# keillernogueira/dynamic-rs-segmentation

Hardware: AMD Instinct MI355X
Metric: training patches/sec dilated_grsl_rate8 64x64x5 (higher is better)
Workload: dtype f32; 1 GPU; dilated_grsl_rate8 (Dilated8Pooling) training step, single_fixed 64x64, 5-band synthetic 2048x2048 tile, global batch 128 (crop+augment+normalise, fwd, loss, bwd, momentum, confusion); global_batch=128, patch=64, bands=5, classes=6, parallelism=dp1, sync_bn=True, rccl_ranks_observed=1

## Files before the change

### dynamic-rs-segmentation_amd/_lib.py

```python
import ctypes as C
import os

_HERE = os.path.dirname(os.path.abspath(__file__))
LIB_PATH = os.path.join(_HERE, "libdrs_hip.so")
DEV_LIB_PATH = os.path.join(_HERE, "libdrs_hip_dev.so")

_p, _i, _f, _d = C.c_void_p, C.c_int, C.c_float, C.c_double
_sz, _u64 = C.c_size_t, C.c_ulonglong

SIGNATURES = {
    "drs_conv_mtile": (_i, [_i]),
    "drs_conv_forward": (_i, [_p, _i, _i, _i, _i, _i, _p, _p, _i, _i, _i, _i, _i, _p, _i, _i, _i, _p, _p]),
    "drs_conv_workspace_floats": (_sz, [_i]),
    "drs_conv_halo_skip": (_i, [_i, _i, _i, _i, _i, _i, _i]),
    "drs_conv_executed_ksteps": (_i, [_i, _i, _i, _i, _i, _i, _i, _p, _p]),
    "drs_conv_forward_ws": (_i, [_p, _i, _i, _i, _i, _i, _p, _p, _i, _i, _i, _i, _i, _p, _i, _i, _i, _p, _p, _sz, _p]),
    "drs_conv_wgrad_splits": (_i, [_i, _i, _i, _i, _i]),
    "drs_conv_wgrad": (_i, [_p, _i, _i, _i, _i, _i, _p, _i, _i, _i, _i, _i, _i, _i, _i, _i, _p, _p, _p]),
    "drs_filter_flip_transpose": (_i, [_p, _p, _i, _i, _i, _p]),
    "drs_filter_pad_cin": (_i, [_p, _p, _i, _i, _i, _i, _p]),
    "drs_split_conv_mtile": (_i, [_i]),
    "drs_split_terms": (_i, [_p, _sz, _i, _p, _p]),
    "drs_filter_split": (_i, [_p, _i, _i, _i, _i, _i, _p, _p, _p]),
    "drs_conv_forward_split": (_i, [_p, _i, _i, _i, _i, _i, _p, _p, _i, _i, _i, _i, _i, _p, _i, _i, _i, _p, _i, _p]),
# ... 91 lines not shown
    "drs_net_se_gate_finish": (_i, [_p, _i, _d, _p]),
    "drs_net_set_two_streams": (_i, [_p, _i]),
    "drs_net_set_class_weights": (_i, [_p, _p, _i]),
    "drs_net_get_class_weights": (_i, [_p, _p, _i, C.POINTER(_i)]),
    "drs_net_set_focal_gamma": (_i, [_p, _f]),
    "drs_net_get_focal_gamma": (_i, [_p, C.POINTER(_f)]),
    "drs_net_timing": (_i, [_p, _i]),
    "drs_net_num_timing_kinds": (_i, []),
    "drs_net_timing_summary": (_i, [_p, _i, C.c_char_p, _i, C.POINTER(_i), C.POINTER(_d), C.POINTER(_d)]),
}
ALLREDUCE_FN = C.CFUNCTYPE(_i, _p, _p, _sz, _i, _i, _p)
WAIT_FN = C.CFUNCTYPE(_i, _p, _i, _p)
WANT_LOGITS, WITH_LABELS, USE_ACC_MASK, USE_LOSS_MASK, NO_UPDATE = 1, 2, 4, 8, 16


DEV_SIGNATURES = {
    "drs_debug_skip_taps": (_i, [_i]), "drs_debug_conv_variant": (_i, [_i]), "drs_debug_conv_wide192": (_i, [_i]),
    "drs_debug_conv_splitk": (_i, [_i]), "drs_debug_conv_hybrid": (_i, [_i]), "drs_debug_conv_sk_order": (_i, [_i]), "drs_debug_conv_prio": (_i, [_i]),
    "drs_debug_conv_sk_geometry": (_i, [_i, _i, _i, _p]), "drs_debug_conv_trace": (_i, [_p]), "drs_debug_conv_lpt": (_i, [_i]), "drs_debug_conv_order": (_i, [_i] * 7 + [_p, _i]),
    "drs_debug_conv_image_tiles": (_i, [_i]), "drs_debug_conv_order_image": (_i, [_i] * 7 + [_p, _i]),
    "drs_debug_wgrad_variant": (_i, [_i]), "drs_debug_wgrad_seg": (_i, [_i]), "drs_debug_wgrad_balance": (_i, [_i]), "drs_debug_wgrad_target": (_i, [_i]),
    "drs_debug_wgrad_target_big": (_i, [_i]), "drs_debug_wgrad_len": (_i, [_i]), "drs_debug_wgrad_minchunks": (_i, [_i]), "drs_debug_wgrad_model": (_i, [_i]), "drs_debug_wgrad_ablate": (_i, [_i]), "drs_debug_wgrad_prio": (_i, [_i]), "drs_debug_cls_variant": (_i, [_i]), "drs_debug_slide_blocks": (_i, [_i]), "drs_debug_slide_minrows": (_i, [_i]), "drs_debug_slide_rowpad": (_i, [_i]), "drs_debug_chain_mode": (_i, [_i]), "drs_debug_jitter": (_i, [C.c_ulonglong]), "drs_debug_wg_stream_prio": (_i, [_i]), "drs_debug_reductions_on_chain": (_i, [_i]), "drs_debug_wgrad_schedule": (_i, [_i, _i, _i]), "drs_debug_variant": (_i, [_i]),
    "drs_debug_wgrad_cut": (_i, [_i] * 7 + [_p, _i, _p, _p]),
}


class DrsError(RuntimeError):
    pass


_lib = None
_dev = None


def _open(path, signatures):
    if not os.path.isfile(path):
        raise DrsError("HIP library not built: %s is missing (run dynamic-rs-segmentation_amd/csrc/build.sh "
                       "or __graft_entry__.build()); there is no CPU fallback" % path)
    import torch
    lib = C.CDLL(path)
    for name, (res, args) in signatures.items():
        fn = getattr(lib, name)
        fn.restype = res
        fn.argtypes = args
    return lib

# ... 49 lines not shown
```

### dynamic-rs-segmentation_amd/csrc/conv_mfma.hip

```cpp
#include "drs_common.hpp"
#include <algorithm>
#include <cstdlib>
#include <map>
#include <mutex>
#include <numeric>
#include <tuple>
#include <vector>

namespace {

constexpr int BK = 32;
constexpr int LDA = BK + 4;

struct ConvArgs {
  const float* in; int S, P, ld_in, coff_in;
  int M;
  const float* w;
  const float* bias;
  float* out; int ld_out, coff_out;
  float* stats;
  int k, rate, pad, Cin, Cout;
  int accumulate;
  int skip_halo;
  float rcpS, rcpSS;
// ... 510 lines not shown
  }
  conv_epilogue<BM, BN, WM, WN>(a, acc, lds, m0, n0);
}

constexpr int WG_MAXT = 64, WG_MAXC = 8;
struct WgradPlan {
  int nclass;
  int n[WG_MAXC];
  int seg_start[WG_MAXC + 1];
  int seg_width[WG_MAXC];
  unsigned char cls[WG_MAXT];
};

struct WgradArgs {
  const float* x; int S, Px, ld_x, coff_x;
  const float* g; int Pg, ld_g, coff_g;
  int M;
  int k, rate, pad, Cin, Cout;
  float* slab;
  int chunks_per_split;
  int ntr, nto;
  int skip_halo;
  int live_cut;
  int prio;
  int ablate;
  float rcpS, rcpSS;
  WgradPlan plan;
#ifdef DRS_DEV
  unsigned long long* trace;
#endif
};

__host__ __device__ __forceinline__ int wave_uniform(int v) {
#if defined(__HIP_DEVICE_COMPILE__)
  return __builtin_amdgcn_readfirstlane(v);
#else
  return v;
#endif
}

__host__ __device__ __forceinline__ void wgrad_assign(const WgradArgs& a, int TR, int id, int& tile, int& split, int& cbeg, int& cend,
                                                      int& live_lo, int& live_hi) {
  const int nchunks_total = (a.M + 31) / 32;
  const int rows_all = a.k * a.k * a.Cin;
  int nr = 0;
  if (a.plan.nclass == 0) {
    const int ntile = a.ntr * a.nto;
    split = id / ntile;
    tile = id % ntile;
  } else {
    int j = 0;
    while (j + 1 < a.plan.nclass && id >= a.plan.seg_start[j + 1]) ++j;
    const int rel = id - a.plan.seg_start[j];
    split = (j ? a.plan.n[j - 1] : 0) + rel / a.plan.seg_width[j];
    const int pos = rel % a.plan.seg_width[j];
    const int want = pos / a.nto;
    int r = 0, seen = 0;
    for (; r < a.ntr; ++r)
      if (a.plan.cls[r] >= j) { if (seen == want) break; ++seen; }
    r = r < a.ntr ? r : a.ntr - 1;
    tile = r * a.nto + pos % a.nto;
    nr = a.plan.n[a.plan.cls[r]];
  }
  tile = wave_uniform(tile);
  split = wave_uniform(split);
  const int R0 = (tile / a.nto) * TR;
  const int rlast = (R0 + TR < rows_all ? R0 + TR : rows_all) - 1;
  int lo, hi;
  live_pixel_range(R0, rlast, a.Cin, a.k, a.rate, a.pad, a.S, a.live_cut, lo, hi);
  if (a.plan.nclass == 0) {
    cbeg = split * a.chunks_per_split;
    cend = cbeg + a.chunks_per_split;
    cend = cend < nchunks_total ? cend : nchunks_total;
  } else {
    const int S2 = a.S * a.S, lp = hi - lo;
    const int live_total = (a.M / S2) * lp;
    const int q = (live_total + nr - 1) / nr;
    auto bound = [&](int s) -> int {
      if (s <= 0) return 0;
      const long long jp = (long long)s * q;
      if (s >= nr || jp >= live_total) return nchunks_total;
      const int img = (int)jp / lp, rem = (int)jp - img * lp;
      return (img * S2 + lo + rem) >> 5;
    };
    cbeg = bound(split);
    cend = bound(split + 1);
  }
  cbeg = wave_uniform(cbeg);
  cend = wave_uniform(cend);
  if (!a.skip_halo) { lo = 0; hi = a.S * a.S; }
  live_lo = lo; live_hi = hi;
}

struct ChunkWalk {
  int c, b, r, y, x0;
  int S, S2, lo, hi, ylo;
  __device__ __forceinline__ void init(int cfirst, int S_, float rcpS, float rcpSS, int lo_, int hi_) {
    S = S_; S2 = S_ * S_; lo = lo_; hi = hi_;
    int q;
    divmod24(lo, S, rcpS, ylo, q);
    c = next_live_chunk(cfirst - 1, S2, rcpSS, lo, hi);
    divmod24(c * 32, S2, rcpSS, b, r);
    divmod24(r, S, rcpS, y, x0);
    c = __builtin_amdgcn_readfirstlane(c); b = __builtin_amdgcn_readfirstlane(b); r = __builtin_amdgcn_readfirstlane(r);
    y = __builtin_amdgcn_readfirstlane(y); x0 = __builtin_amdgcn_readfirstlane(x0); ylo = __builtin_amdgcn_readfirstlane(ylo);
  }
  __device__ __forceinline__ int advance() {
    int r1 = r + 32, b1 = b;
    if (r1 >= S2) { r1 -= S2; ++b1; }
    if ((r1 + 31 >= lo && r1 < hi) || r1 + 31 >= S2 + lo) {
      ++c; r = r1; b = b1;
      x0 += 32;
      if (x0 >= S) { x0 -= S; ++y; }
      if (y >= S) y = 0;
// ... 213 lines not shown
#ifdef DRS_DEV
  if (a.trace && t == 0) a.trace[2 * blockIdx.x + 1] = __builtin_amdgcn_s_memrealtime();
#endif
}

template <int TR, int TO, int MODE>
__global__ __launch_bounds__(64 * (TR >= 64 ? 2 : 1) * (TO >= 64 ? 2 : 1), 3) void wgrad_dma_kernel(const WgradArgs a) {
#if defined(__HIP_DEVICE_COMPILE__)
  constexpr int WR = TR >= 64 ? 2 : 1, WC = TO >= 64 ? 2 : 1;
  constexpr int NW = WR * WC, NT = 64 * NW;
  constexpr int WTR = TR / WR, WTO = TO / WC;
  constexpr int TMr = WTR / 32, TNo = WTO / 32;
  constexpr int BP = 32, HP = 16;
  constexpr int XQ = TR / 4, GQ = TO / 4;
  constexpr int IX = HP * XQ / 64 / NW, IG = HP * GQ / 64 / NW;
  static_assert(IX >= 1 && IG >= 1 && IX * NW * 64 == HP * XQ && IG * NW * 64 == HP * GQ, "tile / wave layout");
  constexpr int XSTAGE = HP * TR, STAGE = HP * (TR + TO);

  __shared__ __attribute__((aligned(1024))) float lds[2 * STAGE];
  __shared__ uint32_t tabx[2][BP], tabg[2][BP];

  constexpr bool AFF = MODE == 1;
  constexpr bool SEG = MODE == 2;
  const int t = threadIdx.x;
  const int lane = t & 63, wave = (AFF || SEG) ? __builtin_amdgcn_readfirstlane(t >> 6) : t >> 6;
  const int li = lane & 31, h = lane >> 5;
  const int wr = wave / WC, wc = wave % WC;

  int tile, split, cbeg, cend, live_lo, live_hi;
#ifdef DRS_DEV
  if (a.trace && t == 0) {
    a.trace[2 * blockIdx.x] = __builtin_amdgcn_s_memrealtime();
    a.trace[32768 + blockIdx.x] = (unsigned long long)__builtin_amdgcn_s_getreg(63492) | ((unsigned long long)__builtin_amdgcn_s_getreg(63508) << 32);
  }
#endif
  wgrad_assign(a, TR, xcd_remap(blockIdx.x, gridDim.x), tile, split, cbeg, cend, live_lo, live_hi);
  const int R0 = (tile / a.nto) * TR;
  const int o0 = (tile % a.nto) * TO;
  const int rows_all = a.k * a.k * a.Cin;
  const int Sxp = a.S + 2 * a.Px, Sgp = a.S + 2 * a.Pg;
  constexpr bool affine = AFF || SEG;
  const int xq = lane % XQ;
  const int myR = R0 + xq * 4;
  const int myRc = myR < rows_all ? myR : 0;
  const int tap = myRc / a.Cin, c0 = myRc % a.Cin;
  const int u = tap / a.k, v = tap % a.k;
  const uint32_t biasx = SEG ? (uint32_t)(32 * a.ld_x) * 4u : 0u, biasg = SEG ? (uint32_t)(32 * a.ld_g) * 4u : 0u;
  const uint32_t xconst = (uint32_t)((a.ablate == 1 ? 0 : (u * a.rate * Sxp + v * a.rate)) * a.ld_x + a.coff_x + c0) * 4u + biasx;
  uint32_t xoff[IX], goff[IG];
  int xpix[IX], gpix[IG];
#pragma unroll
  for (int i = 0; i < IX; ++i) {
    xpix[i] = (64 * (wave + NW * i) + lane) / XQ;
    xoff[i] = xconst + (affine ? (uint32_t)(xpix[i] * a.ld_x) * 4u : 0u);
  }
#pragma unroll
  for (int i = 0; i < IG; ++i) {
    const int f = 64 * (wave + NW * i) + lane;
    gpix[i] = f / GQ;
    goff[i] = (uint32_t)(a.coff_g + o0 + (f % GQ) * 4) * 4u + (affine ? (uint32_t)(gpix[i] * a.ld_g) * 4u : 0u) + biasg;
  }

  f32x16 acc[TMr][TNo];
#pragma unroll
  for (int mi = 0; mi < TMr; ++mi)
#pragma unroll
    for (int ni = 0; ni < TNo; ++ni)
#pragma unroll
      for (int r = 0; r < 16; ++r) acc[mi][ni][r] = 0.f;

  const int nchunks_total = (a.M + BP - 1) / BP;
  const int clast = (a.M & 31) ? nchunks_total - 1 : -1;
  ChunkWalk w;
  w.init(cbeg, a.S, a.rcpS, a.rcpSS, live_lo, live_hi);

  int py = 0, px = 0;
  uint32_t ox = 0, og = 0;
  const uint32_t stepx = (uint32_t)(32 * a.ld_x) * 4u, stepg = (uint32_t)(32 * a.ld_g) * 4u;
  const uint32_t rowjx = (uint32_t)((Sxp - a.S) * a.ld_x) * 4u, rowjg = (uint32_t)((Sgp - a.S) * a.ld_g) * 4u;
  const uint32_t imgjx = (uint32_t)(Sxp * (Sxp - a.S) * a.ld_x) * 4u, imgjg = (uint32_t)(Sgp * (Sgp - a.S) * a.ld_g) * 4u;
  auto pixel_from_index = [&](int p) {
    int pb, rem;
    divmod24(p < a.M ? p : a.M - 1, w.S2, a.rcpSS, pb, rem);
    divmod24(rem, a.S, a.rcpS, py, px);
    ox = (uint32_t)(((pb * Sxp + py + a.Px - a.pad) * Sxp + px + a.Px - a.pad) * a.ld_x) * 4u;
    og = (uint32_t)(((pb * Sgp + py + a.Pg) * Sgp + px + a.Pg) * a.ld_g) * 4u;
  };
  if (!affine && t < BP) pixel_from_index(w.c * BP + t);
  auto fill_tables = [&](int slot, int stepped) {
    if (affine || t >= BP || w.c >= cend) return;
    const int p = w.c * BP + t;
    if (stepped == 1 && p < a.M && a.S >= 11) {
      px += 32; ox += stepx; og += stepg;
      if (a.S >= 32) {
        if (px >= a.S) { px -= a.S; ++py; ox += rowjx; og += rowjg; }
      } else {
#pragma unroll
        for (int k = 0; k < 3; ++k) if (px >= a.S) { px -= a.S; ++py; ox += rowjx; og += rowjg; }
      }
      if (py >= a.S) { py -= a.S; ox += imgjx; og += imgjg; }
    } else if (stepped != 0) {
      pixel_from_index(p);
    }
    tabx[slot][t] = ox;
    tabg[slot][t] = og;
  };

  const char* xbase = reinterpret_cast<const char*>(a.x);
  const char* gbase = reinterpret_cast<const char*>(a.g);
  typedef __attribute__((address_space(3))) void* lds_ptr;
  struct Seg { int brk; int32_t jx, jg; };
  auto chunk_bases = [&](const char*& xb, const char*& gb, Seg& sg) {
    xb = xbase + (size_t)(uint32_t)(((w.b * Sxp + w.y + a.Px - a.pad) * Sxp + w.x0 + a.Px - a.pad) * a.ld_x) * 4u;
    gb = gbase + (size_t)(uint32_t)(((w.b * Sgp + w.y + a.Pg) * Sgp + w.x0 + a.Pg) * a.ld_g) * 4u;
    if (SEG) {
      xb -= biasx; gb -= biasg;
      sg.brk = a.S - w.x0;
      const bool last = w.c == clast, img_end = w.y == a.S - 1;
      sg.jx = last ? -(int32_t)biasx : (int32_t)(rowjx + (img_end ? imgjx : 0u));
      sg.jg = last ? -(int32_t)biasg : (int32_t)(rowjg + (img_end ? imgjg : 0u));
    }
  };
  struct LaneOffsets { uint32_t x[2][IX], g[2][IG]; };
  auto fetch_offsets = [&](int slot, LaneOffsets& o) {
    if (affine) return;
#pragma unroll
    for (int half = 0; half < 2; ++half) {
#pragma unroll
      for (int i = 0; i < IX; ++i) o.x[half][i] = tabx[slot][half * HP + xpix[i]] + xoff[i];
#pragma unroll
      for (int i = 0; i < IG; ++i) o.g[half][i] = tabg[slot][half * HP + gpix[i]] + goff[i];
    }
  };
  auto issue = [&](const char* xb, const char* gb, const Seg& seg, const LaneOffsets& o, int half, int stage) {
    float* sx = lds + stage * STAGE;
    float* sg = sx + XSTAGE;
    if (affine) {
      const char* xh = xb + (size_t)(uint32_t)(half * HP * a.ld_x) * 4u;
      const char* gh = gb + (size_t)(uint32_t)(half * HP * a.ld_g) * 4u;
      int inner = HP;
      if (SEG) {
        const int hb = seg.brk - half * HP;
        if (hb <= 0) { xh += (ptrdiff_t)seg.jx; gh += (ptrdiff_t)seg.jg; }
        else if (hb < HP) inner = hb;
      }
      if (SEG && inner < HP) {
#pragma unroll
        for (int i = 0; i < IX; ++i) {
          uint32_t v = xoff[i] + (xpix[i] >= inner ? (uint32_t)seg.jx : 0u);
          __builtin_amdgcn_global_load_lds(xh + v, (lds_ptr)(sx + (wave + NW * i) * 256), 16, 0, 0);
        }
#pragma unroll
        for (int i = 0; i < IG; ++i) {
          uint32_t v = goff[i] + (gpix[i] >= inner ? (uint32_t)seg.jg : 0u);
          __builtin_amdgcn_global_load_lds(gh + v, (lds_ptr)(sg + (wave + NW * i) * 256), 16, 0, 0);
        }
      } else {
#pragma unroll
        for (int i = 0; i < IX; ++i) {
          uint32_t v = xoff[i]; asm volatile("" : "+v"(v));
          __builtin_amdgcn_global_load_lds(xh + v, (lds_ptr)(sx + (wave + NW * i) * 256), 16, 0, 0);
        }
#pragma unroll
        for (int i = 0; i < IG; ++i) {
          uint32_t v = goff[i]; asm volatile("" : "+v"(v));
          __builtin_amdgcn_global_load_lds(gh + v, (lds_ptr)(sg + (wave + NW * i) * 256), 16, 0, 0);
        }
      }
    } else {
#pragma unroll
      for (int i = 0; i < IX; ++i) __builtin_amdgcn_global_load_lds(xbase + o.x[half][i], (lds_ptr)(sx + (wave + NW * i) * 256), 16, 0, 0);
#pragma unroll
      for (int i = 0; i < IG; ++i) __builtin_amdgcn_global_load_lds(gbase + o.g[half][i], (lds_ptr)(sg + (wave + NW * i) * 256), 16, 0, 0);
    }
  };
  auto zero_tail = [&](int chunk, int half, int stage) {
    if (AFF || chunk != clast) return;
    float* sg = lds + stage * STAGE + XSTAGE;
    for (int e = t; e < HP * TO; e += NT)
      if (chunk * BP + half * HP + e / TO >= a.M) sg[e] = 0.f;
    __syncthreads();
  };
  const int xr = wr * 32 + li, gc = wc * 32 + li;
  constexpr int XG = 32 * WR, GG = 32 * WC;
  auto compute = [&](int stage) {
    const float* Xs = lds + stage * STAGE;
    const float* Gs = Xs + XSTAGE;
    float af[2][TMr], bf[2][TNo];
#pragma unroll
    for (int mi = 0; mi < TMr; ++mi) af[0][mi] = Xs[h * TR + xr + mi * XG];
#pragma unroll
    for (int ni = 0; ni < TNo; ++ni) bf[0][ni] = Gs[h * TO + gc + ni * GG];
#pragma unroll
    for (int s = 0; s < HP / 2; ++s) {
      if (s + 1 < HP / 2) {
#pragma unroll
        for (int mi = 0; mi < TMr; ++mi) af[(s + 1) & 1][mi] = Xs[(2 * s + 2 + h) * TR + xr + mi * XG];
#pragma unroll
        for (int ni = 0; ni < TNo; ++ni) bf[(s + 1) & 1][ni] = Gs[(2 * s + 2 + h) * TO + gc + ni * GG];
        __builtin_amdgcn_sched_group_barrier(0x100, TMr + TNo, 0);
      }
#pragma unroll
      for (int mi = 0; mi < TMr; ++mi)
#pragma unroll
        for (int ni = 0; ni < TNo; ++ni)
          acc[mi][ni] = __builtin_amdgcn_mfma_f32_32x32x2f32(af[s & 1][mi], bf[s & 1][ni], acc[mi][ni], 0, 0, 0);
      __builtin_amdgcn_sched_group_barrier(0x8, TMr * TNo, 0);
    }
  };

  int cA = w.c;
  if (cA < cend) {
    const char *xbA, *gbA, *xbB = xbase, *gbB = gbase;
    LaneOffsets oA, oB;
#pragma unroll
    for (int half = 0; half < 2; ++half) {
#pragma unroll
      for (int i = 0; i < IX; ++i) oA.x[half][i] = oB.x[half][i] = 0u;
#pragma unroll
      for (int i = 0; i < IG; ++i) oA.g[half][i] = oB.g[half][i] = 0u;
    }
    Seg sgA = {32, 0, 0}, sgB = {32, 0, 0};
    chunk_bases(xbA, gbA, sgA);
    fill_tables(0, 0);
    if (!affine) __syncthreads();
    fetch_offsets(0, oA);
    issue(xbA, gbA, sgA, oA, 0, 0);
    int stepped = w.advance();
    int cB = w.c;
    chunk_bases(xbB, gbB, sgB);
    fill_tables(1, stepped);
    asm volatile("s_waitcnt vmcnt(0)" ::: "memory");
    __syncthreads();
    zero_tail(cA, 0, 0);
// ... 287 lines not shown

template <int BM, int BN, int WM, int WN>
int launch_conv(ConvArgs& a, float* ws, size_t ws_floats, hipStream_t st) {
  const int mt = (a.M + BM - 1) / BM, nt = a.Cout / BN;
  if (a.Cin < BK) DRS_LAUNCH((conv_igemm_kernel<BM, BN, WM, WN, true>), dim3(mt * nt), dim3(256), 0, st, a);
  else if constexpr (BM == 128) {
    const bool dma = g_conv_variant != 0;
    if (dma) return launch_conv_dma<BM, BN, WM, WN>(a, ws, ws_floats, st);
    DRS_LAUNCH((conv_igemm_kernel<BM, BN, WM, WN>), dim3(mt * nt), dim3(256), 0, st, a);
  } else DRS_LAUNCH((conv_igemm_kernel<BM, BN, WM, WN>), dim3(mt * nt), dim3(256), 0, st, a);
  return DRS_LAUNCH_CHECK();
}

int g_wgrad_variant = -1;

inline bool wgrad_affine(const WgradArgs& a) { return (a.S & 31) == 0 || a.ablate == 5; }
int g_wgrad_seg = 1;
inline bool wgrad_segments(const WgradArgs& a) {
  const long long Sxp = a.S + 2 * a.Px, Sgp = a.S + 2 * a.Pg, B = a.M / ((long long)a.S * a.S);
  const long long xb = (B * Sxp * Sxp + 64) * a.ld_x * 4, gb = (B * Sgp * Sgp + 64) * a.ld_g * 4;
  return g_wgrad_seg && a.S >= 32 && !wgrad_affine(a) && xb < (1LL << 32) && gb < (1LL << 32);
}

template <int TR, int TO>
int launch_wgrad(const WgradArgs& a, int nwg, hipStream_t st) {
  constexpr int NT = 64 * (TR >= 64 ? 2 : 1) * (TO >= 64 ? 2 : 1);
  const bool dma = g_wgrad_variant < 0 ? (TO == 128 || (TO == 64 && (wgrad_affine(a) || (wgrad_segments(a) && a.M < (1 << 18))))) : g_wgrad_variant == 1;
  if (!dma && wgrad_affine(a)) DRS_LAUNCH((wgrad_kernel<TR, TO, true>), dim3(nwg), dim3(NT), 0, st, a);
  else if (!dma) DRS_LAUNCH((wgrad_kernel<TR, TO, false>), dim3(nwg), dim3(NT), 0, st, a);
  else if (wgrad_affine(a)) DRS_LAUNCH((wgrad_dma_kernel<TR, TO, 1>), dim3(nwg), dim3(NT), 0, st, a);
  else if (wgrad_segments(a)) DRS_LAUNCH((wgrad_dma_kernel<TR, TO, 2>), dim3(nwg), dim3(NT), 0, st, a);
  else DRS_LAUNCH((wgrad_dma_kernel<TR, TO, 0>), dim3(nwg), dim3(NT), 0, st, a);
  return DRS_LAUNCH_CHECK();
}

template <int TR, int TO>
int launch_wgrad_dma_only(const WgradArgs& a, int nwg, hipStream_t st) {
  if (wgrad_affine(a)) DRS_LAUNCH((wgrad_dma_kernel<TR, TO, 1>), dim3(nwg), dim3(256), 0, st, a);
  else if (wgrad_segments(a)) DRS_LAUNCH((wgrad_dma_kernel<TR, TO, 2>), dim3(nwg), dim3(256), 0, st, a);
  else DRS_LAUNCH((wgrad_dma_kernel<TR, TO, 0>), dim3(nwg), dim3(256), 0, st, a);
  return DRS_LAUNCH_CHECK();
}

}

__attribute__((visibility("hidden"))) int drs_step_prep(const StepPrepArgs& a, hipStream_t stream) {
  if (a.n < 0 || a.n > STEP_PREP_MAX) return DRS_ERR_ARG;
  DRS_LAUNCH(step_prep_kernel, dim3(512, a.n + 2), dim3(256), 0, stream, a);
  return DRS_LAUNCH_CHECK();
}


int drs_g_skip_halo_taps = 1;
thread_local int drs_tl_chain = 0;
int drs_g_chain_mode = -1;

namespace {

int g_wgrad_target = 2048;

int pick_tile(int c) { return c % 128 == 0 ? 128 : (c % 64 == 0 ? 64 : 32); }
// ... 41 lines not shown
    return (int)(t > 4096 ? 4096 : t);
  }
  static const int steps[] = {512, 768, 1024, 2048, 3072, 4096};
  int best = steps[0];
  for (int s : steps)
    if (s <= g_wgrad_target && (double)(s > fit ? s : fit) / (s > fit ? fit : s) < (double)(best > fit ? best : fit) / (best > fit ? fit : best)) best = s;
  return best;
}

int wgrad_uniform_splits(int B, int S, int k, int cin, int cout, int len = 0) {
  const long long M = (long long)B * S * S;
  const int tr = pick_wgrad_rows(k * k * cin), to = pick_wgrad_cols(tr, cout);
  const int ntile = ((k * k * cin + tr - 1) / tr) * (cout / to);
  const int nchunks = (int)((M + 31) / 32);
  int want = wgrad_target((long long)nchunks * ntile, ntile, nchunks, false, 4, len) / ntile;
  int maxs = (nchunks + g_wgrad_minchunks - 1) / g_wgrad_minchunks;
  if (maxs < 1) maxs = 1;
  if (want > maxs) want = maxs;
  if (want < 1) want = 1;
  const int cps = (nchunks + want - 1) / want;
  return (nchunks + cps - 1) / cps;
}

bool wgrad_live_plan(int B, int S, int k, int rate, int pad, int cin, int cout, int tr, int to, int cap, WgradPlan& p, int& nwg) {
  const int rows = k * k * cin, ntr = (rows + tr - 1) / tr, nto = cout / to;
  p.nclass = 0;
  if (ntr > WG_MAXT) return false;
  int lp[WG_MAXT], vals[WG_MAXC], nv = 0;
  for (int r = 0; r < ntr; ++r) {
    int lo, hi;
    const int rlast = ((r + 1) * tr < rows ? (r + 1) * tr : rows) - 1;
    live_pixel_range(r * tr, rlast, cin, k, rate, pad, S, 1, lo, hi);
    lp[r] = hi - lo;
    int c = 0;
    while (c < nv && vals[c] != lp[r]) ++c;
    if (c == nv) { if (nv == WG_MAXC) return false; vals[nv++] = lp[r]; }
  }
  if (nv == 1 && vals[0] == S * S) return false;
  for (int i = 1; i < nv; ++i)
    for (int j = i; j > 0 && vals[j] < vals[j - 1]; --j) { const int t = vals[j]; vals[j] = vals[j - 1]; vals[j - 1] = t; }
  int cnt[WG_MAXC] = {0};
  for (int r = 0; r < ntr; ++r) {
    int c = 0;
    while (vals[c] != lp[r]) ++c;
    p.cls[r] = (unsigned char)c;
    ++cnt[c];
  }
  const long long M = (long long)B * S * S;
  const int nchunks = (int)((M + 31) / 32);
  double work = 0;
  for (int c = 0; c < nv; ++c) work += (double)cnt[c] * nto * B * vals[c] / 32.0;
  const int target = wgrad_target((long long)work, ntr * nto, nchunks, true, (tr == 128 && to == 192) ? 3 : 4);
  const double len = work / target;
  int maxs = (nchunks + g_wgrad_minchunks - 1) / g_wgrad_minchunks;
  if (maxs > cap) maxs = cap;
  if (maxs < 1) maxs = 1;
// ... 20 lines not shown
  for (int c = 1; c < nv; ++c)
    if (p.n[c] < p.n[c - 1]) p.n[c] = p.n[c - 1];
  int above = ntr, start = 0;
  for (int j = 0; j < nv; ++j) {
    p.seg_start[j] = start;
    p.seg_width[j] = above * nto;
    start += (p.n[j] - (j ? p.n[j - 1] : 0)) * above * nto;
    above -= cnt[j];
  }
  p.seg_start[nv] = start;
  p.nclass = nv;
  nwg = start;
  return true;
}

int wgrad_bound_splits(int B, int S, int k, int cin, int cout) {
  const int shortest = g_wgrad_len && g_wgrad_len < 96 ? g_wgrad_len : 96;
  const int ua = wgrad_uniform_splits(B, S, k, cin, cout), ub = wgrad_uniform_splits(B, S, k, cin, cout, shortest);
  const int u = ua > ub ? ua : ub;
  int maxs = (int)(((long long)B * S * S + 32LL * g_wgrad_minchunks - 1) / (32LL * g_wgrad_minchunks));
  if (maxs < 1) maxs = 1;
  const int bound = u + u / 2 + 1;
  return bound < maxs ? bound : (maxs > u ? maxs : u);
}

int wgrad_setup(int B, int S, int k, int rate, int pad_before, int cin, int cout, WgradArgs& a, int& nwg, int& tr, int& to, int& nsplit) {
  if ((cin % 32 && cin != 8 && cin != 16) || cout % 32 || B < 1 || S < 1 || k < 1 || rate < 1) return DRS_ERR_ARG;
  const long long M = (long long)B * S * S;
  if (M <= 0 || M >= (1 << 24)) return DRS_ERR_ARG;
  a.x = nullptr; a.g = nullptr; a.slab = nullptr; a.Px = a.Pg = a.ld_x = a.ld_g = a.coff_x = a.coff_g = 0;
  a.S = S; a.M = (int)M;
  a.k = k; a.rate = rate; a.pad = pad_before; a.Cin = cin; a.Cout = cout;
  tr = pick_wgrad_rows(k * k * cin); to = pick_wgrad_cols(tr, cout);
  a.ntr = (k * k * cin + tr - 1) / tr; a.nto = cout / to;
  nsplit = wgrad_uniform_splits(B, S, k, cin, cout);
  const int nchunks = (int)((M + 31) / 32);
  a.chunks_per_split = (nchunks + nsplit - 1) / nsplit;
  a.rcpS = 1.0f / (float)S; a.rcpSS = 1.0f / (float)(S * S);
  a.ablate = g_wgrad_ablate;
  a.prio = g_wgrad_prio >= 0 ? g_wgrad_prio : ((g_wgrad_ablate != 3 && M >= (1LL << 18)) ? 1 : 0);
#ifdef DRS_DEV
  a.trace = g_conv_trace;
#endif
  nwg = nsplit * a.ntr * a.nto;
  a.plan.nclass = 0;
  a.live_cut = 0;
  if (g_wgrad_balance && wgrad_live_plan(B, S, k, rate, pad_before, cin, cout, tr, to, wgrad_bound_splits(B, S, k, cin, cout), a.plan, nwg)) {
    a.live_cut = 1;
    a.skip_halo = drs_g_skip_halo_taps != 0;
  } else {
    a.skip_halo = drs_skip_halo_taps_wgrad(M);
    a.live_cut = a.skip_halo;
  }
  return DRS_OK;
}

int conv_plain_image_g(int B, int S, int k, int rate, int cin, int cout) {
  if (cin < 32 || cin % 32) return 0;
  const int bn = pick_conv_tile(cout, cin);
  if (bn < 64) return 0;
  const int mt = (int)(((long long)B * S * S + 127) / 128), nt = cout / bn;
  if (sk_geometry(mt * nt, k * k * (cin / 32), bn, 2ull * (size_t)sk_max_w() * 128 * (size_t)bn).G) return 0;
  return conv_image_tiles_g(B, S, k, rate, cin, cout);
}

}

extern "C" {

#ifdef DRS_DEV
// ... 147 lines not shown
    default:  return launch_conv<256, 32, 4, 1>(a, workspace, workspace_floats, st);
  }
}

int drs_conv_forward(const float* in, int B, int S, int P, int ld_in, int coff_in, const float* w, const float* bias,
                     int k, int rate, int pad_before, int cin, int cout, float* out, int ld_out, int coff_out,
                     int accumulate, float* stats_partial, void* stream) {
  return drs_conv_forward_ws(in, B, S, P, ld_in, coff_in, w, bias, k, rate, pad_before, cin, cout, out, ld_out, coff_out, accumulate,
                             stats_partial, nullptr, 0, stream);
}

int drs_conv_wgrad_splits(int B, int S, int k, int cin, int cout) { return wgrad_bound_splits(B, S, k, cin, cout); }

#ifdef DRS_DEV
int drs_debug_wgrad_cut(int B, int S, int k, int rate, int pad_before, int cin, int cout, int* out, int cap, int* out_tile_splits,
                        int* out_tile_rows) {
  WgradArgs a;
  int nwg, tr, to, nsplit;
  if (wgrad_setup(B, S, k, rate, pad_before, cin, cout, a, nwg, tr, to, nsplit)) return -1;
  if (out_tile_rows) *out_tile_rows = tr;
  for (int r = 0; r < a.ntr && out_tile_splits; ++r) out_tile_splits[r] = a.plan.nclass ? a.plan.n[a.plan.cls[r]] : nsplit;
  for (int i = 0; i < nwg && i < cap && out; ++i) {
    int tile, split, cbeg, cend, lo, hi;
    wgrad_assign(a, tr, i, tile, split, cbeg, cend, lo, hi);
    out[5 * i] = tile / a.nto; out[5 * i + 1] = tile % a.nto; out[5 * i + 2] = split; out[5 * i + 3] = cbeg; out[5 * i + 4] = cend;
  }
  return nwg;
}
#endif

int drs_conv_wgrad(const float* x, int B, int S, int Px, int ld_x, int coff_x, const float* g, int Pg, int ld_g,
                   int coff_g, int k, int rate, int pad_before, int cin, int cin_real, int cout, float* slab,
                   float* grad, void* stream) {
  if (!x || !g || !slab || !grad || cin_real > cin) return DRS_ERR_ARG;
  if ((long long)B * (S + 2 * Px) * (S + 2 * Px) * ld_x >= (1LL << 30)) return DRS_ERR_ARG;
  if ((long long)B * (S + 2 * Pg) * (S + 2 * Pg) * ld_g >= (1LL << 30)) return DRS_ERR_ARG;
  WgradArgs a;
  int nwg, tr, to, nsplit;
  if (wgrad_setup(B, S, k, rate, pad_before, cin, cout, a, nwg, tr, to, nsplit)) return DRS_ERR_ARG;
  a.x = x; a.Px = Px; a.ld_x = ld_x; a.coff_x = coff_x;
  a.g = g; a.Pg = Pg; a.ld_g = ld_g; a.coff_g = coff_g; a.slab = slab;
  hipStream_t st = (hipStream_t)stream;
  int rc;
  if (tr == 128 && to == 192) rc = launch_wgrad_dma_only<128, 192>(a, nwg, st);
  else if (tr == 128 && to == 128) rc = launch_wgrad<128, 128>(a, nwg, st);
  else if (tr == 128 && to == 64) rc = launch_wgrad<128, 64>(a, nwg, st);
  else if (tr == 128 && to == 32) rc = launch_wgrad<128, 32>(a, nwg, st);
  else if (tr == 64 && to == 128) rc = launch_wgrad<64, 128>(a, nwg, st);
  else if (tr == 64 && to == 64) rc = launch_wgrad<64, 64>(a, nwg, st);
  else if (tr == 64 && to == 32) rc = launch_wgrad<64, 32>(a, nwg, st);
// ... 28 lines not shown
```

### dynamic-rs-segmentation_amd/csrc/drs_common.hpp

```cpp
#pragma once
#include <hip/hip_runtime.h>
#include <stdint.h>

#define DRS_OK 0
#define DRS_ERR_ARG 1
#define DRS_ERR_HIP 2

typedef float f32x4 __attribute__((ext_vector_type(4)));
typedef float f32x16 __attribute__((ext_vector_type(16)));

struct ActView {
  float* base;
  int S;
  int P;
  int ld;
  int coff;
  uint16_t* terms;
  int nt;
};

__device__ __forceinline__ void view_store4(const ActView& v, size_t e, f32x4 x) {
  if (v.base) *reinterpret_cast<f32x4*>(v.base + e) = x;
  if (v.terms) {
    uint16_t* t = v.terms + (e & ~(size_t)31) * v.nt + (e & 31);
// ... 62 lines not shown
  u_hi = u_hi < k ? u_hi : k;
  v_hi = v_hi < k ? v_hi : k;
  if (u_lo >= u_hi || v_lo >= v_hi) { u_lo = v_lo = 0; u_hi = v_hi = k; }
}
__host__ __device__ __forceinline__ int image_tile_pos(int mt, int S, int g, int& y, int& x0) {
  const int Pc = 128 >> g, npc = S / Pc;
  const int t2 = mt / npc;
  x0 = (mt - t2 * npc) * Pc;
  const int grp = t2 / S;
  y = t2 - grp * S;
  return grp;
}

__host__ __device__ __forceinline__ void live_pixel_range(int row_first, int row_last, int Cin, int k, int rate, int pad, int S, int enable,
                                                          int& lo, int& hi) {
  const int dy_min = (row_first / Cin / k) * rate - pad, dy_max = (row_last / Cin / k) * rate - pad;
  int ylo = -dy_max > 0 ? -dy_max : 0;
  int yhi = S - dy_min < S ? S - dy_min : S;
  if (!enable || ylo >= yhi) { ylo = 0; yhi = S; }
  lo = ylo * S;
  hi = yhi * S;
}

__device__ __forceinline__ int next_live_chunk(int c, int S2, float rcpSS, int lo, int hi) {
  const int p = 32 * (c + 1);
  int b, r;
  divmod24(p, S2, rcpSS, b, r);
  if (r + 31 >= lo && r < hi) return c + 1;
  if (r + 31 >= S2 + lo) return c + 1;
  return ((r < lo ? b : b + 1) * S2 + lo) >> 5;
}

template <int NSLOT, int WM, int BN, class Col, class LaneSum, class Each>
__device__ __forceinline__ void tile_column_stats(float* red, int t, int wm, bool writer, float n_tile, Col col, LaneSum lanesum,
                                                  Each each, float* dst) {
  float* red2 = red + WM * BN;
#pragma unroll
  for (int ni = 0; ni < NSLOT; ++ni) {
    float s = 0.f;
    each(ni, [&](float v) { s += v; });
    s = lanesum(s);
    if (writer) red[wm * BN + col(ni)] = s;
  }
  __syncthreads();
  const float rn = 1.0f / n_tile;
#pragma unroll
// ... 45 lines not shown
```

### include/drs_dev.h

```cpp
#ifndef DRS_DEV_H_
#define DRS_DEV_H_
#ifdef __cplusplus
extern "C" {
#endif

int drs_debug_skip_taps(int v);
int drs_debug_conv_variant(int v);
int drs_debug_conv_wide192(int v);
int drs_debug_conv_lpt(int v);
int drs_debug_conv_order(int B, int S, int k, int rate, int pad_before, int cin, int cout, int* out, int cap);
int drs_debug_conv_image_tiles(int g);
int drs_debug_conv_order_image(int B, int S, int k, int rate, int pad_before, int cin, int cout, int* out, int cap);
int drs_debug_conv_trace(void* dev_buffer);
int drs_debug_conv_splitk(int v);
int drs_debug_conv_hybrid(int v);
int drs_debug_conv_sk_order(int v);
int drs_debug_conv_prio(int v);
int drs_debug_conv_sk_geometry(int tiles, int nks, int bn, int* out3);
int drs_debug_wgrad_variant(int v);
int drs_debug_wgrad_seg(int v);
int drs_debug_wgrad_balance(int v);
int drs_debug_wgrad_target(int v);
int drs_debug_wgrad_target_big(int v);
int drs_debug_wgrad_len(int v);
int drs_debug_wgrad_minchunks(int v);
int drs_debug_wgrad_prio(int v);
int drs_debug_wgrad_ablate(int v);
int drs_debug_wgrad_model(int v);
int drs_debug_slide_blocks(int v);
int drs_debug_slide_minrows(int v);
int drs_debug_jitter(unsigned long long seed);
int drs_debug_wg_stream_prio(int arm);
int drs_debug_reductions_on_chain(int on);
int drs_debug_wgrad_schedule(int layer_slabs, int streams, int defer);
int drs_debug_chain_mode(int v);
int drs_debug_slide_rowpad(int v);
int drs_debug_cls_variant(int v);
int drs_debug_variant(int v);
int drs_debug_wgrad_cut(int B, int S, int k, int rate, int pad_before, int cin, int cout, int* out, int cap, int* out_tile_splits,
                        int* out_tile_rows);

#ifdef __cplusplus
}
#endif
#endif
```

Baseline: 2712 patches/s.

## Restrict dilated-conv weight-gradient pixel walk to a 2D live window

Adds a windowed mode to the DMA weight-gradient kernel. For each row tile it computes the rectangular region of output pixels whose dilated taps land inside the image, in both y and x, instead of only a range of rows. Split balancing and the staged loads then walk only that window, using row and image jumps and zeroing the tail stage. The mode is enabled by default only for three layer shapes at batch 128 and patch 64, which adds a hardcoded shape table and a new code path in the kernel.

```diff
diff --git a/dynamic-rs-segmentation_amd/_lib.py b/dynamic-rs-segmentation_amd/_lib.py
--- a/dynamic-rs-segmentation_amd/_lib.py
+++ b/dynamic-rs-segmentation_amd/_lib.py
@@ -137,6 +137,7 @@
     "drs_debug_wgrad_variant": (_i, [_i]), "drs_debug_wgrad_seg": (_i, [_i]), "drs_debug_wgrad_balance": (_i, [_i]), "drs_debug_wgrad_target": (_i, [_i]),
     "drs_debug_wgrad_target_big": (_i, [_i]), "drs_debug_wgrad_len": (_i, [_i]), "drs_debug_wgrad_minchunks": (_i, [_i]), "drs_debug_wgrad_model": (_i, [_i]), "drs_debug_wgrad_ablate": (_i, [_i]), "drs_debug_wgrad_prio": (_i, [_i]), "drs_debug_cls_variant": (_i, [_i]), "drs_debug_slide_blocks": (_i, [_i]), "drs_debug_slide_minrows": (_i, [_i]), "drs_debug_slide_rowpad": (_i, [_i]), "drs_debug_chain_mode": (_i, [_i]), "drs_debug_jitter": (_i, [C.c_ulonglong]), "drs_debug_wg_stream_prio": (_i, [_i]), "drs_debug_reductions_on_chain": (_i, [_i]), "drs_debug_wgrad_schedule": (_i, [_i, _i, _i]), "drs_debug_variant": (_i, [_i]),
     "drs_debug_wgrad_cut": (_i, [_i] * 7 + [_p, _i, _p, _p]),
+    "drs_debug_wgrad_window": (_i, [_i]), "drs_debug_wgrad_executed": (_i, [_i] * 7 + [_p, _p]),
 }
 
 
diff --git a/dynamic-rs-segmentation_amd/csrc/conv_mfma.hip b/dynamic-rs-segmentation_amd/csrc/conv_mfma.hip
--- a/dynamic-rs-segmentation_amd/csrc/conv_mfma.hip
+++ b/dynamic-rs-segmentation_amd/csrc/conv_mfma.hip
@@ -556,6 +556,7 @@
   int ntr, nto;
   int skip_halo;
   int live_cut;
+  int window;
   int prio;
   int ablate;
   float rcpS, rcpSS;
@@ -573,8 +574,9 @@
 #endif
 }
 
-__host__ __device__ __forceinline__ void wgrad_assign(const WgradArgs& a, int TR, int id, int& tile, int& split, int& cbeg, int& cend,
-                                                      int& live_lo, int& live_hi) {
+template <bool WIN>
+__host__ __device__ __forceinline__ void wgrad_assign_t(const WgradArgs& a, int TR, int id, int& tile, int& split, int& cbeg, int& cend,
+                                                        int& live_lo, int& live_hi, LiveWindow& win) {
   const int nchunks_total = (a.M + 31) / 32;
   const int rows_all = a.k * a.k * a.Cin;
   int nr = 0;
@@ -602,18 +604,20 @@
   const int rlast = (R0 + TR < rows_all ? R0 + TR : rows_all) - 1;
   int lo, hi;
   live_pixel_range(R0, rlast, a.Cin, a.k, a.rate, a.pad, a.S, a.live_cut, lo, hi);
+  if (WIN) win = live_pixel_window(R0, rlast, a.Cin, a.k, a.rate, a.pad, a.S, a.live_cut);
   if (a.plan.nclass == 0) {
     cbeg = split * a.chunks_per_split;
     cend = cbeg + a.chunks_per_split;
     cend = cend < nchunks_total ? cend : nchunks_total;
   } else {
-    const int S2 = a.S * a.S, lp = hi - lo;
+    const int S2 = a.S * a.S, lp = WIN ? win.nrows * win.W : hi - lo;
     const int live_total = (a.M / S2) * lp;
     const int q = (live_total + nr - 1) / nr;
     auto bound = [&](int s) -> int {
       if (s <= 0) return 0;
       const long long jp = (long long)s * q;
       if (s >= nr || jp >= live_total) return nchunks_total;
+      if (WIN) return window_pixel_at((int)jp, a.S, win) >> 5;
       const int img = (int)jp / lp, rem = (int)jp - img * lp;
       return (img * S2 + lo + rem) >> 5;
     };
@@ -624,6 +628,12 @@
   cend = wave_uniform(cend);
   if (!a.skip_halo) { lo = 0; hi = a.S * a.S; }
   live_lo = lo; live_hi = hi;
+  if (WIN && !a.skip_halo) { win.ylo = 0; win.nrows = a.S; win.xlo = 0; win.W = a.S; }
+}
+__host__ __device__ __forceinline__ void wgrad_assign(const WgradArgs& a, int TR, int id, int& tile, int& split, int& cbeg, int& cend,
+                                                      int& live_lo, int& live_hi) {
+  LiveWindow win;
+  wgrad_assign_t<false>(a, TR, id, tile, split, cbeg, cend, live_lo, live_hi, win);
 }
 
 struct ChunkWalk {
@@ -883,24 +893,26 @@
 
   constexpr bool AFF = MODE == 1;
   constexpr bool SEG = MODE == 2;
+  constexpr bool WIN = MODE == 3;
   const int t = threadIdx.x;
-  const int lane = t & 63, wave = (AFF || SEG) ? __builtin_amdgcn_readfirstlane(t >> 6) : t >> 6;
+  const int lane = t & 63, wave = (AFF || SEG || WIN) ? __builtin_amdgcn_readfirstlane(t >> 6) : t >> 6;
   const int li = lane & 31, h = lane >> 5;
   const int wr = wave / WC, wc = wave % WC;
 
   int tile, split, cbeg, cend, live_lo, live_hi;
+  LiveWindow win;
 #ifdef DRS_DEV
   if (a.trace && t == 0) {
     a.trace[2 * blockIdx.x] = __builtin_amdgcn_s_memrealtime();
     a.trace[32768 + blockIdx.x] = (unsigned long long)__builtin_amdgcn_s_getreg(63492) | ((unsigned long long)__builtin_amdgcn_s_getreg(63508) << 32);
   }
 #endif
-  wgrad_assign(a, TR, xcd_remap(blockIdx.x, gridDim.x), tile, split, cbeg, cend, live_lo, live_hi);
+  wgrad_assign_t<WIN>(a, TR, xcd_remap(blockIdx.x, gridDim.x), tile, split, cbeg, cend, live_lo, live_hi, win);
   const int R0 = (tile / a.nto) * TR;
   const int o0 = (tile % a.nto) * TO;
   const int rows_all = a.k * a.k * a.Cin;
   const int Sxp = a.S + 2 * a.Px, Sgp = a.S + 2 * a.Pg;
-  constexpr bool affine = AFF || SEG;
+  constexpr bool affine = AFF || SEG || WIN;
   const int xq = lane % XQ;
   const int myR = R0 + xq * 4;
   const int myRc = myR < rows_all ? myR : 0;
@@ -933,7 +945,8 @@
   const int nchunks_total = (a.M + BP - 1) / BP;
   const int clast = (a.M & 31) ? nchunks_total - 1 : -1;
   ChunkWalk w;
-  w.init(cbeg, a.S, a.rcpS, a.rcpSS, live_lo, live_hi);
+  if (!WIN) w.init(cbeg, a.S, a.rcpS, a.rcpSS, live_lo, live_hi);
+  else { w.c = w.b = w.r = w.y = w.x0 = 0; w.S = a.S; w.S2 = a.S * a.S; w.lo = w.hi = w.ylo = 0; }
 
   int py = 0, px = 0;
   uint32_t ox = 0, og = 0;
@@ -970,7 +983,7 @@
   const char* xbase = reinterpret_cast<const char*>(a.x);
   const char* gbase = reinterpret_cast<const char*>(a.g);
   typedef __attribute__((address_space(3))) void* lds_ptr;
-  struct Seg { int brk; int32_t jx, jg; };
+  struct Seg { int brk; int32_t jx, jg; int valid; };
   auto chunk_bases = [&](const char*& xb, const char*& gb, Seg& sg) {
     xb = xbase + (size_t)(uint32_t)(((w.b * Sxp + w.y + a.Px - a.pad) * Sxp + w.x0 + a.Px - a.pad) * a.ld_x) * 4u;
     gb = gbase + (size_t)(uint32_t)(((w.b * Sgp + w.y + a.Pg) * Sgp + w.x0 + a.Pg) * a.ld_g) * 4u;
@@ -1005,7 +1018,21 @@
         if (hb <= 0) { xh += (ptrdiff_t)seg.jx; gh += (ptrdiff_t)seg.jg; }
         else if (hb < HP) inner = hb;
       }
-      if (SEG && inner < HP) {
+      if (WIN && seg.brk < HP) inner = seg.brk;
+      if (WIN && seg.valid < HP) {
+#pragma unroll
+        for (int i = 0; i < IX; ++i) {
+          uint32_t v = xoff[i] + (xpix[i] >= inner ? (uint32_t)seg.jx : 0u);
+          if (xpix[i] >= seg.valid) v = xoff[i] - (uint32_t)(xpix[i] * a.ld_x) * 4u;
+          __builtin_amdgcn_global_load_lds(xh + v, (lds_ptr)(sx + (wave + NW * i) * 256), 16, 0, 0);
+        }
+#pragma unroll
+        for (int i = 0; i < IG; ++i) {
+          uint32_t v = goff[i] + (gpix[i] >= inner ? (uint32_t)seg.jg : 0u);
+          if (gpix[i] >= seg.valid) v = goff[i] - (uint32_t)(gpix[i] * a.ld_g) * 4u;
+          __builtin_amdgcn_global_load_lds(gh + v, (lds_ptr)(sg + (wave + NW * i) * 256), 16, 0, 0);
+        }
+      } else if ((SEG || WIN) && inner < HP) {
 #pragma unroll
         for (int i = 0; i < IX; ++i) {
           uint32_t v = xoff[i] + (xpix[i] >= inner ? (uint32_t)seg.jx : 0u);
@@ -1036,7 +1063,7 @@
     }
   };
   auto zero_tail = [&](int chunk, int half, int stage) {
-    if (AFF || chunk != clast) return;
+    if (AFF || WIN || chunk != clast) return;
     float* sg = lds + stage * STAGE + XSTAGE;
     for (int e = t; e < HP * TO; e += NT)
       if (chunk * BP + half * HP + e / TO >= a.M) sg[e] = 0.f;
@@ -1070,7 +1097,64 @@
     }
   };
 
-  int cA = w.c;
+  if constexpr (WIN) {
+    const int pend = cend * BP < a.M ? cend * BP : a.M;
+    const int qbeg = __builtin_amdgcn_readfirstlane(window_pixels_before(cbeg * BP, a.S, win));
+    const int qend = __builtin_amdgcn_readfirstlane(window_pixels_before(pend, a.S, win));
+    const int nst = (qend - qbeg + HP - 1) / HP;
+    const int lastvalid = qend - qbeg - (nst - 1) * HP;
+    const int lpw = win.nrows * win.W;
+    int sb = qbeg / lpw, sy = (qbeg - sb * lpw) / win.W, sx = qbeg - sb * lpw - sy * win.W;
+    sb = __builtin_amdgcn_readfirstlane(sb); sy = __builtin_amdgcn_readfirstlane(sy); sx = __builtin_amdgcn_readfirstlane(sx);
+    const int32_t wrowjx = (int32_t)((Sxp - win.W) * a.ld_x) * 4, wrowjg = (int32_t)((Sgp - win.W) * a.ld_g) * 4;
+    const int32_t wimgjx = (int32_t)(Sxp * (Sxp - win.nrows) * a.ld_x) * 4, wimgjg = (int32_t)(Sgp * (Sgp - win.nrows) * a.ld_g) * 4;
+    auto next_stage = [&](int s, const char*& xb, const char*& gb, Seg& sg) {
+      if (s >= nst) { sg.valid = 0; return; }
+      const int y = win.ylo + sy, x = win.xlo + sx;
+      xb = xbase + (size_t)(uint32_t)(((sb * Sxp + y + a.Px - a.pad) * Sxp + x + a.Px - a.pad) * a.ld_x) * 4u;
+      gb = gbase + (size_t)(uint32_t)(((sb * Sgp + y + a.Pg) * Sgp + x + a.Pg) * a.ld_g) * 4u;
+      const bool img_end = sy == win.nrows - 1;
+      sg.brk = win.W - sx;
+      sg.jx = wrowjx + (img_end ? wimgjx : 0);
+      sg.jg = wrowjg + (img_end ? wimgjg : 0);
+      sg.valid = s == nst - 1 ? lastvalid : HP;
+      sx += HP;
+      if (sx >= win.W) { sx -= win.W; if (++sy >= win.nrows) { sy = 0; ++sb; } }
+    };
+    auto zero_tail_win = [&](int valid, int stage) {
+      if (valid >= HP) return;
+      float* sg = lds + stage * STAGE + XSTAGE;
+      for (int e = t; e < HP * TO; e += NT)
+        if (e / TO >= valid) sg[e] = 0.f;
+      __syncthreads();
+    };
+    if (nst > 0) {
+      const char *xb, *gb;
+      Seg sg = {HP, 0, 0, HP};
+      LaneOffsets od = {};
+      next_stage(0, xb, gb, sg);
+      issue(xb, gb, sg, od, 0, 0);
+      asm volatile("s_waitcnt vmcnt(0)" ::: "memory");
+      __syncthreads();
+      zero_tail_win(sg.valid, 0);
+      int quart = -1;
+      for (int s = 0; s < nst; s += 2) {
+        if (a.prio) set_prio_by_progress(s, nst, quart, a.prio);
+        next_stage(s + 1, xb, gb, sg);
+        issue(xb, gb, sg, od, 0, 1);
+        compute(0);
+        asm volatile("s_waitcnt vmcnt(0)" ::: "memory");
+        __syncthreads();
+        zero_tail_win(sg.valid, 1);
+        if (s + 2 < nst) { next_stage(s + 2, xb, gb, sg); issue(xb, gb, sg, od, 0, 0); }
+        compute(1);
+        asm volatile("s_waitcnt vmcnt(0)" ::: "memory");
+        __syncthreads();
+        if (s + 2 < nst) zero_tail_win(sg.valid, 0);
+      }
+    }
+  }
+  int cA = WIN ? cend : w.c;
   if (cA < cend) {
     const char *xbA, *gbA, *xbB = xbase, *gbB = gbase;
     LaneOffsets oA, oB;
@@ -1404,9 +1488,14 @@
   return g_wgrad_seg && a.S >= 32 && !wgrad_affine(a) && xb < (1LL << 32) && gb < (1LL << 32);
 }
 
+constexpr bool wgrad_window_tile(int tr, int to) { return tr >= 64 && to >= 64; }
+
 template <int TR, int TO>
 int launch_wgrad(const WgradArgs& a, int nwg, hipStream_t st) {
   constexpr int NT = 64 * (TR >= 64 ? 2 : 1) * (TO >= 64 ? 2 : 1);
+  if constexpr (wgrad_window_tile(TR, TO)) {
+    if (a.window) { DRS_LAUNCH((wgrad_dma_kernel<TR, TO, 3>), dim3(nwg), dim3(NT), 0, st, a); return DRS_LAUNCH_CHECK(); }
+  }
   const bool dma = g_wgrad_variant < 0 ? (TO == 128 || (TO == 64 && (wgrad_affine(a) || (wgrad_segments(a) && a.M < (1 << 18))))) : g_wgrad_variant == 1;
   if (!dma && wgrad_affine(a)) DRS_LAUNCH((wgrad_kernel<TR, TO, true>), dim3(nwg), dim3(NT), 0, st, a);
   else if (!dma) DRS_LAUNCH((wgrad_kernel<TR, TO, false>), dim3(nwg), dim3(NT), 0, st, a);
@@ -1418,7 +1507,8 @@
 
 template <int TR, int TO>
 int launch_wgrad_dma_only(const WgradArgs& a, int nwg, hipStream_t st) {
-  if (wgrad_affine(a)) DRS_LAUNCH((wgrad_dma_kernel<TR, TO, 1>), dim3(nwg), dim3(256), 0, st, a);
+  if (a.window) DRS_LAUNCH((wgrad_dma_kernel<TR, TO, 3>), dim3(nwg), dim3(256), 0, st, a);
+  else if (wgrad_affine(a)) DRS_LAUNCH((wgrad_dma_kernel<TR, TO, 1>), dim3(nwg), dim3(256), 0, st, a);
   else if (wgrad_segments(a)) DRS_LAUNCH((wgrad_dma_kernel<TR, TO, 2>), dim3(nwg), dim3(256), 0, st, a);
   else DRS_LAUNCH((wgrad_dma_kernel<TR, TO, 0>), dim3(nwg), dim3(256), 0, st, a);
   return DRS_LAUNCH_CHECK();
@@ -1506,7 +1596,7 @@
   return (nchunks + cps - 1) / cps;
 }
 
-bool wgrad_live_plan(int B, int S, int k, int rate, int pad, int cin, int cout, int tr, int to, int cap, WgradPlan& p, int& nwg) {
+bool wgrad_live_plan(int B, int S, int k, int rate, int pad, int cin, int cout, int tr, int to, int cap, bool window, WgradPlan& p, int& nwg) {
   const int rows = k * k * cin, ntr = (rows + tr - 1) / tr, nto = cout / to;
   p.nclass = 0;
   if (ntr > WG_MAXT) return false;
@@ -1516,6 +1606,7 @@
     const int rlast = ((r + 1) * tr < rows ? (r + 1) * tr : rows) - 1;
     live_pixel_range(r * tr, rlast, cin, k, rate, pad, S, 1, lo, hi);
     lp[r] = hi - lo;
+    if (window) { const LiveWindow w = live_pixel_window(r * tr, rlast, cin, k, rate, pad, S, 1); lp[r] = w.nrows * w.W; }
     int c = 0;
     while (c < nv && vals[c] != lp[r]) ++c;
     if (c == nv) { if (nv == WG_MAXC) return false; vals[nv++] = lp[r]; }
@@ -1582,6 +1673,25 @@
   if (maxs < 1) maxs = 1;
   const int bound = u + u / 2 + 1;
   return bound < maxs ? bound : (maxs > u ? maxs : u);
+}
+
+int g_wgrad_window = 1;
+
+int wgrad_window_rule(int B, int S, int k, int rate, int cin, int cout) {
+  if (B != 128 || S != 64) return 0;
+  struct Row { int k, rate, cin, cout; };
+  static const Row gains[] = {{4, 4, 128, 128},
+                              {3, 6, 192, 192},
+                              {3, 8, 256, 256}};
+  for (const Row& r : gains)
+    if (r.k == k && r.rate == rate && r.cin == cin && r.cout == cout) return 1;
+  return 0;
+}
+
+bool wgrad_window_wanted(int B, int S, int k, int rate, int pad, int cin, int cout, int tr, int to) {
+  if (g_wgrad_window == 0 || (g_wgrad_window == 1 && !wgrad_window_rule(B, S, k, rate, cin, cout))) return false;
+  (void)pad;
+  return S >= 32 && S % 2 == 0 && k > 1 && cin % 32 == 0 && wgrad_window_tile(tr, to) && g_wgrad_variant != 0 && g_wgrad_ablate == 0;
 }
 
 int wgrad_setup(int B, int S, int k, int rate, int pad_before, int cin, int cout, WgradArgs& a, int& nwg, int& tr, int& to, int& nsplit) {
@@ -1605,7 +1715,17 @@
   nwg = nsplit * a.ntr * a.nto;
   a.plan.nclass = 0;
   a.live_cut = 0;
-  if (g_wgrad_balance && wgrad_live_plan(B, S, k, rate, pad_before, cin, cout, tr, to, wgrad_bound_splits(B, S, k, cin, cout), a.plan, nwg)) {
+  a.window = 0;
+  if (g_wgrad_balance && wgrad_window_wanted(B, S, k, rate, pad_before, cin, cout, tr, to) &&
+      wgrad_live_plan(B, S, k, rate, pad_before, cin, cout, tr, to, wgrad_bound_splits(B, S, k, cin, cout), true, a.plan, nwg)) {
+    a.window = 1;
+    a.live_cut = 1;
+    a.skip_halo = drs_g_skip_halo_taps != 0;
+    return DRS_OK;
+  }
+  nwg = nsplit * a.ntr * a.nto;
+  a.plan.nclass = 0;
+  if (g_wgrad_balance && wgrad_live_plan(B, S, k, rate, pad_before, cin, cout, tr, to, wgrad_bound_splits(B, S, k, cin, cout), false, a.plan, nwg)) {
     a.live_cut = 1;
     a.skip_halo = drs_g_skip_halo_taps != 0;
   } else {
@@ -1799,10 +1919,42 @@
   for (int r = 0; r < a.ntr && out_tile_splits; ++r) out_tile_splits[r] = a.plan.nclass ? a.plan.n[a.plan.cls[r]] : nsplit;
   for (int i = 0; i < nwg && i < cap && out; ++i) {
     int tile, split, cbeg, cend, lo, hi;
-    wgrad_assign(a, tr, i, tile, split, cbeg, cend, lo, hi);
+    LiveWindow win;
+    if (a.window) wgrad_assign_t<true>(a, tr, i, tile, split, cbeg, cend, lo, hi, win);
+    else wgrad_assign(a, tr, i, tile, split, cbeg, cend, lo, hi);
     out[5 * i] = tile / a.nto; out[5 * i + 1] = tile % a.nto; out[5 * i + 2] = split; out[5 * i + 3] = cbeg; out[5 * i + 4] = cend;
   }
   return nwg;
+}
+
+int drs_debug_wgrad_window(int v) { const int old = g_wgrad_window; if (v >= 0) g_wgrad_window = v; return old; }
+
+int drs_debug_wgrad_executed(int B, int S, int k, int rate, int pad_before, int cin, int cout, long long* stages_executed,
+                             long long* stages_all) {
+  WgradArgs a;
+  int nwg, tr, to, nsplit;
+  if (!stages_executed || !stages_all || wgrad_setup(B, S, k, rate, pad_before, cin, cout, a, nwg, tr, to, nsplit)) return DRS_ERR_ARG;
+  long long ex = 0, all = 0;
+  const int S2 = S * S;
+  for (int i = 0; i < nwg; ++i) {
+    int tile, split, cbeg, cend, lo, hi;
+    LiveWindow win;
+    if (a.window) {
+      wgrad_assign_t<true>(a, tr, i, tile, split, cbeg, cend, lo, hi, win);
+      const int pend = cend * 32 < a.M ? cend * 32 : a.M;
+      ex += (window_pixels_before(pend, S, win) - window_pixels_before(cbeg * 32, S, win) + 15) / 16;
+      all += (pend - cbeg * 32 + 15) / 16;
+    } else {
+      wgrad_assign(a, tr, i, tile, split, cbeg, cend, lo, hi);
+      for (int c = cbeg; c < cend; ++c) {
+        const int r = (c * 32) % S2;
+        ex += 2 * ((r + 31 >= lo && r < hi) || r + 31 >= S2 + lo);
+      }
+      all += 2LL * (cend - cbeg);
+    }
+  }
+  *stages_executed = ex; *stages_all = all;
+  return DRS_OK;
 }
 #endif
 
diff --git a/dynamic-rs-segmentation_amd/csrc/drs_common.hpp b/dynamic-rs-segmentation_amd/csrc/drs_common.hpp
--- a/dynamic-rs-segmentation_amd/csrc/drs_common.hpp
+++ b/dynamic-rs-segmentation_amd/csrc/drs_common.hpp
@@ -108,6 +108,42 @@
   hi = yhi * S;
 }
 
+struct LiveWindow { int ylo, nrows, xlo, W; };
+__host__ __device__ __forceinline__ LiveWindow live_pixel_window(int row_first, int row_last, int Cin, int k, int rate, int pad, int S, int enable) {
+  int lo, hi;
+  live_pixel_range(row_first, row_last, Cin, k, rate, pad, S, enable, lo, hi);
+  LiveWindow w;
+  w.ylo = lo / S; w.nrows = hi / S - w.ylo; w.xlo = 0; w.W = S;
+  const int t0 = row_first / Cin, t1 = row_last / Cin;
+  if (!enable || (S & 1) || t1 - t0 + 1 >= k) return w;
+  int xlo = S, xhi = 0;
+  for (int t = t0; t <= t1; ++t) {
+    const int dx = (t % k) * rate - pad;
+    const int a = -dx > 0 ? -dx : 0, b = S - dx < S ? S - dx : S;
+    if (a < b) { xlo = a < xlo ? a : xlo; xhi = b > xhi ? b : xhi; }
+  }
+  xlo &= ~1;
+  xhi += (xhi - xlo) & 1;
+  if (xhi - xlo < 16 || xhi > S) return w;
+  w.xlo = xlo; w.W = xhi - xlo;
+  return w;
+}
+__host__ __device__ __forceinline__ int window_pixels_before(int P, int S, const LiveWindow& w) {
+  const int S2 = S * S, img = P / S2, rem = P - img * S2, y = rem / S, x = rem - y * S;
+  int n = img * w.nrows * w.W;
+  if (y >= w.ylo + w.nrows) n += w.nrows * w.W;
+  else if (y >= w.ylo) {
+    int c = x - w.xlo;
+    c = c < 0 ? 0 : (c > w.W ? w.W : c);
+    n += (y - w.ylo) * w.W + c;
+  }
+  return n;
+}
+__host__ __device__ __forceinline__ int window_pixel_at(int q, int S, const LiveWindow& w) {
+  const int lp = w.nrows * w.W, img = q / lp, rem = q - img * lp, yy = rem / w.W;
+  return img * S * S + (w.ylo + yy) * S + w.xlo + (rem - yy * w.W);
+}
+
 __device__ __forceinline__ int next_live_chunk(int c, int S2, float rcpSS, int lo, int hi) {
   const int p = 32 * (c + 1);
   int b, r;
diff --git a/include/drs_dev.h b/include/drs_dev.h
--- a/include/drs_dev.h
+++ b/include/drs_dev.h
@@ -39,6 +39,9 @@
 int drs_debug_variant(int v);
 int drs_debug_wgrad_cut(int B, int S, int k, int rate, int pad_before, int cin, int cout, int* out, int cap, int* out_tile_splits,
                         int* out_tile_rows);
+int drs_debug_wgrad_window(int v);
+int drs_debug_wgrad_executed(int B, int S, int k, int rate, int pad_before, int cin, int cout, long long* stages_executed,
+                             long long* stages_all);
 
 #ifdef __cplusplus
 }
```

Result: no change. 2727 patches/s (median of 6 runs) (+0.6%).
